# cambridge-mlg/RECOMBINER

Measured on AMD Instinct MI355X. Metric: INRs trained/sec (whole node) + PSNR@bpp vs reference, CIFAR-10, higher is better.
Workload: dtype bf16

## Files before the change

include/rcb.h:

```cpp
#ifndef RCB_H_
#define RCB_H_

#include <stdint.h>

#ifdef __cplusplus
extern "C" {
#endif

#define RCB_VERSION 406
#define RCB_OK 0
#define RCB_ERR_ARG (-1)
#define RCB_ERR_SHAPE (-2)
#define RCB_ERR_UNSUPPORTED (-3)
#define RCB_KL_SLOTS 1024
#define RCB_KL_FX_SCALE 16777216.0

typedef void* rcb_stream_t;

int rcb_version(void);
const char* rcb_last_error_string(void);
#define RCB_STRUCT_SIREN_DESC 0
#define RCB_STRUCT_LEVEL 1
#define RCB_STRUCT_LEVEL_BWD 2
#define RCB_STRUCT_ADAM_CFG 3
#define RCB_STRUCT_ADAM_TENSOR 4
#define RCB_STRUCT_REC_DESC 5
int64_t rcb_struct_bytes(int32_t which);

typedef struct {
  int32_t n_rows;
  int32_t samples;
  int32_t n_pix;
  int32_t fourier_dim;
  int32_t pe_dim;
  int32_t n_hidden;
  int32_t hidden;
  int32_t out_dim;
  int64_t xf_inr_stride;
  int64_t w_row_stride;
  float   w0;
  int32_t precision;
  int32_t pe_bf16;
// ... 98 lines not shown
  void* next_out_bf16;
  int64_t next_ld_bf16;
  uint64_t rng_seed;
  const int64_t* rng_step_dev;
  int64_t rng_step_add;
  uint32_t rng_stream;
  uint32_t eps_from_rng;
  uint64_t rng_group_offset;
  void* next_out_lo;
  float* sample_sum_ws;
  const int32_t* col_map;
} rcb_level_bwd;

int rcb_posterior_bwd(const rcb_level_bwd* lv, const rcb_adam_cfg* adam, rcb_stream_t stream);

int rcb_adam_flat(float* p, const float* g, float* m, float* v, int64_t n, const rcb_adam_cfg* cfg,
                  rcb_stream_t stream);

#define RCB_ADAM_MAX_TENSORS 16
typedef struct {
  float* p;
  const float* g;
  float* m;
  float* v;
  int64_t n;
} rcb_adam_tensor;
int rcb_adam_multi(const rcb_adam_tensor* tensors, int32_t count, const rcb_adam_cfg* cfg, rcb_stream_t stream);

int rcb_debug_generic_kernels_only(int32_t on);

#define RCB_ATRANS_MAX_LAYERS 8
#define RCB_ATRANS_PLAN_HEAD 12
int64_t rcb_atrans_pack_elems(int32_t n_layers, const int32_t* sizes);
int rcb_atrans_pack(const float* const* A, int32_t n_layers, const int32_t* sizes, void* packed, int32_t want_lo,
                    rcb_stream_t stream);
int rcb_atrans_plan(int64_t rows, int32_t n_layers, const int32_t* sizes, int32_t n_cu, int32_t* plan, int32_t max_ints);
int rcb_atrans_apply(const float* x, int64_t ld_x, const void* x_hi, const void* x_lo, int64_t ld_x16, float* out,
                     int64_t ld_out, int64_t rows, int32_t n_layers, const int32_t* sizes, const void* packed, int32_t transpose,
                     int32_t terms, const int32_t* plan_dev, const int32_t* plan_head, float* workspace, rcb_stream_t stream);
int64_t rcb_atrans_workspace_floats(int64_t rows, int32_t n_layers, const int32_t* sizes, const int32_t* plan_head);
int64_t rcb_atrans_wgrad_narrow_workspace(int32_t L, int32_t n_slabs);
int rcb_atrans_wgrad_narrow(const float* h, const void* h_hi, const void* h_lo, int64_t ld_h, const float* d, const void* d_hi,
                            const void* d_lo, int64_t ld_d, int64_t rows, int32_t L, float* dA, float* workspace,
                            int32_t n_slabs, rcb_stream_t stream);

int rcb_step_begin(const float* adam_table, int64_t n_steps, const int64_t* step, float* dyn, int64_t* kl_slots,
                   rcb_stream_t stream);
int rcb_step_end(const float* sse, int32_t n_sse, double mse_scale, const int64_t* kl_slots, double* mse_log,
                 double* kl_log, int64_t n_log, int64_t* step, int64_t* aux_counter ,
                 rcb_stream_t stream);

#define RCB_MOM_FX_SCALE 1073741824.0
#define RCB_MOM_FX_LO_SCALE 4294967296.0
int rcb_col_moments(const float* loc, const float* log_scale, int32_t rows, int32_t cols, int64_t* out_fx,
                    rcb_stream_t stream);

#define RCB_REC_EXACT 0
#define RCB_REC_FAST 1

typedef struct rcb_rec_desc {
  const float* loc;
  const float* scale;
  const float* p_loc;
  const float* p_scale;
  int32_t rows, cols;
  const float* const* tables_t;
// ... 82 lines not shown
```

recombiner_amd/_lib.py:

```python
import ctypes as C
import os

import torch

_HERE = os.path.dirname(os.path.abspath(__file__))
LIB_PATH = os.environ.get("RCB_LIB") or os.path.join(_HERE, "lib", "librcb_hip.so")

EXPORTS = ["rcb_version", "rcb_last_error_string", "rcb_struct_bytes", "rcb_siren_fwd", "rcb_siren_bwd", "rcb_siren_loss_bwd",
           "rcb_reparam_fwd", "rcb_gauss_kl", "rcb_beta_update", "rcb_posterior_bwd", "rcb_adam_flat",
           "rcb_col_moments", "rcb_rec_score_argmax", "rcb_rec_commit", "rcb_rec_workspace_bytes", "rcb_softplus_scale", "rcb_gauss_kl_colsum", "rcb_upconv_fwd",
           "rcb_upconv_dgrad", "rcb_upconv_wgrad", "rcb_upconv_wgrad_workspace", "rcb_adam_multi", "rcb_step_begin",
           "rcb_step_end", "rcb_upconv_weff_build", "rcb_upconv_weff_grad",
           "rcb_upconv_dgrad_partial_rows", "rcb_debug_generic_kernels_only", "rcb_philox_normal",
           "rcb_reparam_rng_fwd", "rcb_upconv_bwd_fused", "rcb_tile_gather", "rcb_tile_crop", "rcb_tile_fold",
           "rcb_window_gather", "rcb_window_fold", "rcb_siren_reduce_chunks", "rcb_phaseconv_pack", "rcb_phaseconv_pack_uint4",
           "rcb_phaseconv_fwd", "rcb_phaseconv_dgrad", "rcb_phaseconv_wgrad", "rcb_phaseconv_wgrad_workspace",
           "rcb_phase_bigweight", "rcb_phase_bigweight_grad", "rcb_atrans_pack_elems", "rcb_atrans_pack", "rcb_atrans_plan",
           "rcb_atrans_apply", "rcb_atrans_workspace_floats", "rcb_atrans_wgrad_narrow_workspace", "rcb_atrans_wgrad_narrow",
           "rcb_stage1_1d_fwd", "rcb_stage1_1d_dgrad", "rcb_stage1_1d_wgrad", "rcb_stage1_1d_wgrad_workspace",
           "rcb_reparam_hier_rng_fwd", "rcb_debug_siren_wave_tiles"]


class RcbError(RuntimeError):
    pass


class SirenDesc(C.Structure):
    _fields_ = [("n_rows", C.c_int32), ("samples", C.c_int32), ("n_pix", C.c_int32), ("fourier_dim", C.c_int32),
                ("pe_dim", C.c_int32), ("n_hidden", C.c_int32), ("hidden", C.c_int32), ("out_dim", C.c_int32),
                ("xf_inr_stride", C.c_int64), ("w_row_stride", C.c_int64), ("w0", C.c_float),
                ("precision", C.c_int32), ("pe_bf16", C.c_int32), ("dw_bf16", C.c_void_p), ("pixel_chunks", C.c_int32),
                ("xf_bf16", C.c_void_p), ("pe_grid_dims", C.c_int32), ("pe_patch_nums", C.c_int32 * 3),
                ("pe_patch_size", C.c_int32 * 3), ("dw_bf16_stride", C.c_int64), ("hidden_dims", C.c_int32 * 4),
                ("dw_lo", C.c_void_p), ("clock_probe", C.c_void_p)]


class Level(C.Structure):
    _fields_ = [("loc", C.c_void_p), ("log_scale", C.c_void_p), ("enc_sample", C.c_void_p),
                ("enc_mask", C.c_void_p), ("row_map", C.c_void_p), ("row_perm", C.c_void_p),
                ("col_map", C.c_void_p), ("eps", C.c_void_p), ("rows", C.c_int32), ("cols", C.c_int32),
                ("cols_out", C.c_int32), ("scale_is_sigma", C.c_int32), ("mu_sigma_ws", C.c_void_p)]


class RecDesc(C.Structure):
    _fields_ = [("loc", C.c_void_p), ("scale", C.c_void_p), ("p_loc", C.c_void_p), ("p_scale", C.c_void_p),
                ("rows", C.c_int32), ("cols", C.c_int32), ("tables_t", C.c_void_p), ("table_absmax", C.c_void_p),
                ("max_glen", C.c_int32), ("gumbel", C.c_void_p), ("gumbel_absmax", C.c_double),
                ("n_candidates", C.c_int32), ("job_row", C.c_void_p), ("job_start", C.c_void_p),
                ("job_glen", C.c_void_p), ("n_jobs", C.c_int32)]


class AdamTensor(C.Structure):
    _fields_ = [("p", C.c_void_p), ("g", C.c_void_p), ("m", C.c_void_p), ("v", C.c_void_p), ("n", C.c_int64)]


class AdamCfg(C.Structure):
    _fields_ = [("lr", C.c_float), ("beta1", C.c_float), ("beta2", C.c_float), ("eps", C.c_float),
                ("step", C.c_int32), ("dyn_scalars", C.c_void_p)]


class LevelBwd(C.Structure):
    _fields_ = [("loc", C.c_void_p), ("log_scale", C.c_void_p), ("enc_mask", C.c_void_p), ("p_loc", C.c_void_p),
                ("p_scale", C.c_void_p), ("p_scale_is_log", C.c_int32), ("beta", C.c_void_p),
                ("group_idx", C.c_void_p), ("n_groups", C.c_int32), ("kl_scalar", C.c_float),
                ("d_out", C.c_void_p), ("eps", C.c_void_p), ("member_ptr", C.c_void_p),
                ("member_idx", C.c_void_p), ("row_perm_inv", C.c_void_p), ("col_inv", C.c_void_p),
                ("rows", C.c_int32), ("cols", C.c_int32), ("cols_out", C.c_int32), ("samples", C.c_int32),
                ("g_loc", C.c_void_p), ("g_log_scale", C.c_void_p), ("m_loc", C.c_void_p), ("v_loc", C.c_void_p),
                ("m_ls", C.c_void_p), ("v_ls", C.c_void_p), ("kl_accum", C.c_void_p), ("kl_scalar_dev", C.c_void_p),
                ("next_out", C.c_void_p), ("next_eps", C.c_void_p), ("next_out_bf16", C.c_void_p),
                ("next_ld_bf16", C.c_int64), ("rng_seed", C.c_uint64), ("rng_step_dev", C.c_void_p),
                ("rng_step_add", C.c_int64), ("rng_stream", C.c_uint32), ("eps_from_rng", C.c_uint32),
                ("rng_group_offset", C.c_uint64), ("next_out_lo", C.c_void_p), ("sample_sum_ws", C.c_void_p), ("col_map", C.c_void_p)]


_lib = None
ABI_VERSION = 406
_MIRRORS = {0: SirenDesc, 1: Level, 2: LevelBwd, 3: AdamCfg, 4: AdamTensor, 5: RecDesc}


def load():
    global _lib
    if _lib is None:
        if not os.path.exists(LIB_PATH):
            raise RcbError(f"{LIB_PATH} not found: run `python -m recombiner_amd.build` (no CPU fallback exists)")
        lib = C.CDLL(LIB_PATH)
        lib.rcb_last_error_string.restype = C.c_char_p
        lib.rcb_upconv_wgrad_workspace.restype = C.c_int64
        lib.rcb_rec_workspace_bytes.restype = C.c_int64
        lib.rcb_phaseconv_pack_uint4.restype = C.c_int64
        lib.rcb_phaseconv_wgrad_workspace.restype = C.c_int64
        lib.rcb_stage1_1d_wgrad_workspace.restype = C.c_int64
        lib.rcb_atrans_pack_elems.restype = C.c_int64
        lib.rcb_atrans_wgrad_narrow_workspace.restype = C.c_int64
        lib.rcb_atrans_workspace_floats.restype = C.c_int64
        for name in EXPORTS:
            if not hasattr(lib, name):
                raise RcbError(f"{LIB_PATH} does not export {name}")
        lib.rcb_struct_bytes.restype = C.c_int64
        if lib.rcb_version() != ABI_VERSION:
            raise RcbError(f"{LIB_PATH} is ABI version {lib.rcb_version()}, this binding was written against {ABI_VERSION}: "
                           "rebuild with `python -m recombiner_amd.build --force`")
        for which, cls in _MIRRORS.items():
            if lib.rcb_struct_bytes(which) != C.sizeof(cls):
                raise RcbError(f"{cls.__name__}: the library's structure has {lib.rcb_struct_bytes(which)} bytes, the ctypes "
                               f"mirror {C.sizeof(cls)} -- _lib.py has drifted from include/rcb.h")
        _lib = lib
    return _lib


# ... 29 lines not shown
```

recombiner_amd/csrc/atrans.hip:

```cpp
#include "rcb_common.h"

#include <algorithm>
#include <type_traits>
#include <vector>

using namespace rcb;

namespace {

typedef __bf16 bf16x8 __attribute__((ext_vector_type(8)));
typedef float f32x16 __attribute__((ext_vector_type(16)));
typedef float f32x4 __attribute__((ext_vector_type(4)));

#ifndef ATRANS_DIAG
#define ATRANS_DIAG 0
#endif
#ifndef ATRANS_STAMPS
#define ATRANS_STAMPS 0
#endif
#ifndef ATRANS_SPREAD_PIN
#define ATRANS_SPREAD_PIN 1
#endif
constexpr int BM = 256, BK = 32, NT = 512, MAXL = RCB_ATRANS_MAX_LAYERS, MAXSEG = 7;
constexpr int XT_BYTES = BM * BK * 4;

__device__ __forceinline__ constexpr int rho(int r, int h) { return (r & 3) + 8 * (r >> 2) + 4 * h; }
__device__ __forceinline__ int xswz(int row, int c) { return row * 128 + ((c ^ ((row >> 1) & 7)) << 4); }
__device__ __forceinline__ int bswz(int row, int c) { return row * 64 + ((c ^ ((row >> 2) & 3)) << 4); }

typedef __attribute__((address_space(3))) void* lds_ptr_t;
__device__ __forceinline__ void dma16(const void* g, char* l) {
  __builtin_amdgcn_global_load_lds(g, (lds_ptr_t)l, 16, 0, 0);
}
__device__ __forceinline__ f32x16 mma(bf16x8 a, bf16x8 b, f32x16 c) {
#if ATRANS_DIAG == 4
  asm volatile("" ::"v"(a), "v"(b));
  return c;
#else
  return __builtin_amdgcn_mfma_f32_32x32x16_bf16(a, b, c, 0, 0, 0);
#endif
}
template <int N>
__device__ __forceinline__ void wait_vm() { asm volatile("s_waitcnt vmcnt(%0)" ::"n"(N) : "memory"); }
#if ATRANS_STAMPS
__device__ unsigned long long g_stamps[8][40][6];
#define STAMP(it, pt)                                                                 \
  do {                                                                               \
    if (blockIdx.x == 0 && (it) < 40) {                                              \
      const unsigned long long t_ = __builtin_amdgcn_s_memtime();                    \
      if (lane == 0) g_stamps[wave][it][pt] = t_;                                    \
    }                                                                                \
  } while (0)
#else
#define STAMP(it, pt)
#endif

struct AtArgs {
  const float* x;
  const __bf16* xh;
  const __bf16* xl;
  long long ld_x16;
  float* out;
  long long ld_x, ld_out, rows;
  int n_layers;
  int L[MAXL], Lp[MAXL], off[MAXL];
  const __bf16* bh[MAXL];
  const __bf16* bl[MAXL];
  const int4* segs;
  const int* seg_begin;
  int n_wg;
  int nt_out;
  float* ws;
  long long ld_ws;
};

template <int NCB, int TERMS>
struct Geo {
  static constexpr int NBW = (2 * NCB + 7) / 8;
  static constexpr int NDMA = 4 + NBW * (TERMS == 3 ? 2 : 1);
  static constexpr int BH_OFF = XT_BYTES;
  static constexpr int BT_BYTES = NCB * 32 * BK * 2;
  static constexpr int BL_OFF = BH_OFF + BT_BYTES;
  static constexpr int STAGE = BH_OFF + (TERMS == 3 ? 2 : 1) * BT_BYTES;
  static constexpr int NSTAGE = TERMS == 3 ? 2 : 3;
};
constexpr int LDS_MAX_BYTES = 3 * (XT_BYTES + MAXSEG * 32 * BK * 2);

template <int NCB, int TERMS, bool RAGGED, bool PLANES>
__device__ __forceinline__ void run_segment(const AtArgs& a, const int4 sg, const int4 sk, char* __restrict__ lds) {
  typedef Geo<NCB, TERMS> G;
  const int t = threadIdx.x, lane = t & 63;
  const int wave = __builtin_amdgcn_readfirstlane(t >> 6);
  const int l = sg.x, row0 = sg.y, cb0 = sg.z, ncb = sg.w;
  const int K = a.L[l], Lp = a.Lp[l];
  const int kc0 = sk.x, nk = sk.y - sk.x;
  const __bf16* __restrict__ bh = a.bh[l];
  const __bf16* __restrict__ bl = a.bl[l];
  const float* __restrict__ xl0 = PLANES ? nullptr : a.x + a.off[l];

  f32x16 acc[NCB];
#pragma unroll
  for (int i = 0; i < NCB; ++i)
#pragma unroll
    for (int q = 0; q < 16; ++q) acc[i][q] = 0.f;

  const float* xsrc[4];
  const __bf16* psrc[4];
  int xk[4];
#pragma unroll
  for (int i = 0; i < 4; ++i) {
    if (PLANES) {
      const int row = 32 * wave + 16 * (i & 1) + (lane >> 2);
      const int c = (lane & 3) ^ ((row >> 2) & 3);
      const long long gr = min((long long)row0 + row, a.rows - 1);
      psrc[i] = ((i >> 1) ? a.xl : a.xh) + gr * a.ld_x16 + a.off[l];
      xk[i] = 8 * c;
      xsrc[i] = nullptr;
    } else {
      const int row = 32 * wave + 8 * i + (lane >> 3);
      const int c = (lane & 7) ^ ((row >> 1) & 7);
      const long long gr = min((long long)row0 + row, a.rows - 1);
      xsrc[i] = xl0 + gr * a.ld_x;
      xk[i] = 4 * c;
      psrc[i] = nullptr;
    }
  }
  const __bf16* bsrc[G::NBW];
  const __bf16* bsrc2[G::NBW];
  int bdst[G::NBW];
#pragma unroll
  for (int j = 0; j < G::NBW; ++j) {
    const int d = min(wave + 8 * j, 2 * NCB - 1);
    const int row = 16 * d + (lane >> 2);
    const int c = (lane & 3) ^ ((row >> 2) & 3);
    const int grow = min(cb0 * 32 + row, Lp - 1);
    bsrc[j] = bh + (long long)grow * Lp + 8 * c;
    bsrc2[j] = bl + (long long)grow * Lp + 8 * c;
    bdst[j] = __builtin_amdgcn_readfirstlane(d * 1024);
  }
  auto issue_one = [&](int kc_, int i) {
    char* __restrict__ st = lds + (kc_ % G::NSTAGE) * G::STAGE;
    const int kc = ATRANS_DIAG == 2 ? 0 : kc0 + kc_;
    if (i < 4) {
      if (PLANES) {
        const int k = RAGGED ? 0 : min(kc * BK + xk[i], K - 8);
        dma16(psrc[i] + k, st + (i >> 1) * (XT_BYTES / 2) + (32 * wave + 16 * (i & 1)) * 64);
      } else {
        const int k = RAGGED ? 0 : min(kc * BK + xk[i], K - 4);
        dma16(xsrc[i] + k, st + (32 * wave + 8 * i) * 128);
      }
    } else if (TERMS == 3) {
      const int j = (i - 4) >> 1;
      if ((i - 4) & 1) dma16(bsrc2[j] + kc * BK, st + G::BL_OFF + bdst[j]);
      else dma16(bsrc[j] + kc * BK, st + G::BH_OFF + bdst[j]);
    } else {
      dma16(bsrc[i - 4] + kc * BK, st + G::BH_OFF + bdst[i - 4]);
    }
  };
  auto issue = [&](int kc) {
#pragma unroll
    for (int i = 0; i < G::NDMA; ++i) issue_one(kc, i);
  };

  const int frow = lane & 31, fh = lane >> 5;
  const int xrow = 32 * wave + frow;
  bf16x8 xh[2], xlo[2];
  f32x4 raw[4];
  auto x_read = [&](const char* __restrict__ st) {
    if (PLANES) {
#pragma unroll
      for (int q = 0; q < 4; ++q)
        if (TERMS >= 2 || q < 2)
          raw[q] = *reinterpret_cast<const f32x4*>(st + (q >> 1) * (XT_BYTES / 2) + bswz(xrow, 2 * (q & 1) + fh));
    } else {
#pragma unroll
      for (int q = 0; q < 4; ++q) raw[q] = *reinterpret_cast<const f32x4*>(st + xswz(xrow, 4 * (q >> 1) + 2 * fh + (q & 1)));
    }
  };
  auto x_convert = [&](int q) {
    if (PLANES) {
      if (q < 2) xh[q] = __builtin_bit_cast(bf16x8, raw[q]);
      else if (TERMS >= 2) xlo[q - 2] = __builtin_bit_cast(bf16x8, raw[q]);
      return;
    }
#pragma unroll
    for (int i = 0; i < 4; ++i) {
      const float v = raw[q][i];
      const __bf16 hb = (__bf16)v;
      xh[q >> 1][4 * (q & 1) + i] = hb;
      if (TERMS >= 2) xlo[q >> 1][4 * (q & 1) + i] = (__bf16)(v - (float)hb);
    }
  };
  constexpr int NBT = G::NDMA - 4;
  constexpr int CBR = (NCB - 1) / 2;
  auto compute = [&](const char* __restrict__ cur, const char* __restrict__ nxt, int kn, auto issue_c, auto pref_c) {
    constexpr bool ISSUE = decltype(issue_c)::value, PREF = decltype(pref_c)::value;
    bf16x8 b0 = *reinterpret_cast<const bf16x8*>(cur + G::BH_OFF + bswz(frow, fh));
    bf16x8 b1 = *reinterpret_cast<const bf16x8*>(cur + G::BH_OFF + bswz(frow, 2 + fh));
#pragma unroll
    for (int cb = 0; cb < NCB; ++cb) {
      const bf16x8 c0 = b0, c1 = b1;
      if (cb + 1 < NCB) {
        b0 = *reinterpret_cast<const bf16x8*>(cur + G::BH_OFF + bswz((cb + 1) * 32 + frow, fh));
        b1 = *reinterpret_cast<const bf16x8*>(cur + G::BH_OFF + bswz((cb + 1) * 32 + frow, 2 + fh));
      }
      acc[cb] = mma(xh[0], c0, acc[cb]);
// ... 19 lines not shown
        }
      }
#if ATRANS_SPREAD_PIN
      __builtin_amdgcn_sched_barrier(0);
#endif
    }
    if (PREF) {
      STAMP(kn - 2, 4);
#pragma unroll
      for (int q = 0; q < 4; ++q) x_convert(q);
    }
  };
  auto yes = std::integral_constant<bool, true>{};
  auto no = std::integral_constant<bool, false>{};

  if (RAGGED) {
    for (int kr = 0; kr < nk; ++kr) {
      const int kc = kc0 + kr;
      __syncthreads();
#pragma unroll
      for (int j = 0; j < G::NBW; ++j) {
        dma16(bsrc[j] + kc * BK, lds + G::BH_OFF + bdst[j]);
        if (TERMS == 3) dma16(bsrc2[j] + kc * BK, lds + G::BL_OFF + bdst[j]);
      }
#pragma unroll
      for (int i = 0; i < 4; ++i) {
        const int k0 = kc * BK + xk[i];
        if (PLANES) {
          const int row = 32 * wave + 16 * (i & 1) + (lane >> 2), pc = lane & 3;
          const bool rok = (long long)row0 + row < a.rows;
          bf16x8 v;
#pragma unroll
          for (int e = 0; e < 8; ++e) v[e] = (rok && k0 + e < K) ? psrc[i][k0 + e] : (__bf16)0.f;
          *reinterpret_cast<bf16x8*>(lds + (i >> 1) * (XT_BYTES / 2) + row * 64 + pc * 16) = v;
        } else {
          const int row = 32 * wave + 8 * i + (lane >> 3), pc = lane & 7;
          const bool rok = (long long)row0 + row < a.rows;
          f32x4 v;
#pragma unroll
          for (int e = 0; e < 4; ++e) v[e] = (rok && k0 + e < K) ? xsrc[i][k0 + e] : 0.f;
          *reinterpret_cast<f32x4*>(lds + row * 128 + pc * 16) = v;
        }
      }
      wait_vm<0>();
      __syncthreads();
      x_read(lds);
#pragma unroll
      for (int q = 0; q < 4; ++q) x_convert(q);
      compute(lds, lds, -1, no, no);
    }
    __syncthreads();
  } else if (G::NSTAGE == 2) {
    issue(0);
    for (int kc = 0; kc < nk; ++kc) {
      wait_vm<0>();
      __builtin_amdgcn_s_barrier();
      __builtin_amdgcn_sched_barrier(0);
      const char* cur = lds + (kc & 1) * G::STAGE;
      x_read(cur);
#pragma unroll
      for (int q = 0; q < 4; ++q) x_convert(q);
      if (kc + 1 < nk) compute(cur, cur, kc + 1, yes, no);
      else compute(cur, cur, -1, no, no);
    }
    __builtin_amdgcn_s_barrier();
  } else {
    issue(0);
// ... 5 lines not shown
    }
    x_read(lds);
#pragma unroll
    for (int q = 0; q < 4; ++q) x_convert(q);
    int kc = 0;
    for (; kc + 2 < nk; ++kc) {
      STAMP(kc, 0);
      wait_vm<G::NDMA>();
      STAMP(kc, 1);
      __builtin_amdgcn_s_barrier();
      __builtin_amdgcn_sched_barrier(0);
      STAMP(kc, 2);
      if (ATRANS_DIAG != 3) compute(lds + (kc % 3) * G::STAGE, lds + ((kc + 1) % 3) * G::STAGE, kc + 2, yes, yes);
      else issue(kc + 2);
      STAMP(kc, 5);
    }
    if (kc + 1 < nk) {
      wait_vm<G::NDMA>();
      __builtin_amdgcn_s_barrier();
      __builtin_amdgcn_sched_barrier(0);
      if (ATRANS_DIAG != 3) compute(lds + (kc % 3) * G::STAGE, lds + ((kc + 1) % 3) * G::STAGE, -1, no, yes);
      ++kc;
    }
    wait_vm<0>();
    __builtin_amdgcn_s_barrier();
    __builtin_amdgcn_sched_barrier(0);
    if (ATRANS_DIAG != 3) compute(lds + (kc % 3) * G::STAGE, lds, -1, no, no);
    __builtin_amdgcn_s_barrier();
  }

  const bool direct = sk.z < 0;
  float* __restrict__ ob = (direct ? a.out : a.ws + (long long)sk.z * a.rows * a.ld_ws) + a.off[l];
  const long long ldo = direct ? a.ld_out : a.ld_ws;
#pragma unroll
  for (int cb = 0; cb < NCB; ++cb) {
    if (cb < ncb && (ATRANS_DIAG != 1 || a.rows < 0)) {
      const int col = (cb0 + cb) * 32 + frow;
      if (col < K) {
#pragma unroll
        for (int q = 0; q < 16; ++q) {
          const long long row = (long long)row0 + 32 * wave + rho(q, fh);
          if (row < a.rows) {
            if (a.nt_out) __builtin_nontemporal_store(acc[cb][q], ob + row * ldo + col);
            else ob[row * ldo + col] = acc[cb][q];
          }
        }
      }
    }
  }
}

template <int TERMS, bool RAGGED, bool PLANES>
__device__ __forceinline__ void dispatch_upto4(const AtArgs& a, const int4 sg, const int4 sk, char* lds) {
  switch (sg.w) {
    case 1: run_segment<1, TERMS, RAGGED, PLANES>(a, sg, sk, lds); break;
    case 2: run_segment<2, TERMS, RAGGED, PLANES>(a, sg, sk, lds); break;
    case 3: run_segment<3, TERMS, RAGGED, PLANES>(a, sg, sk, lds); break;
    default: run_segment<4, TERMS, RAGGED, PLANES>(a, sg, sk, lds); break;
  }
}

template <int TERMS, bool RAGGED, bool PLANES>
__device__ __forceinline__ void dispatch_segment(const AtArgs& a, const int4 sg, const int4 sk, char* lds) {
  if constexpr (TERMS == 3) {
    if (sg.w > 4) {
      const int n1 = (sg.w + 1) / 2;
      dispatch_upto4<TERMS, RAGGED, PLANES>(a, make_int4(sg.x, sg.y, sg.z, n1), sk, lds);
      dispatch_upto4<TERMS, RAGGED, PLANES>(a, make_int4(sg.x, sg.y, sg.z + n1, sg.w - n1), sk, lds);
    } else {
      dispatch_upto4<TERMS, RAGGED, PLANES>(a, sg, sk, lds);
    }
    return;
  }
  switch (sg.w) {
    case 1: run_segment<1, TERMS, RAGGED, PLANES>(a, sg, sk, lds); break;
    case 2: run_segment<2, TERMS, RAGGED, PLANES>(a, sg, sk, lds); break;
    case 3: run_segment<3, TERMS, RAGGED, PLANES>(a, sg, sk, lds); break;
    case 4: run_segment<4, TERMS, RAGGED, PLANES>(a, sg, sk, lds); break;
    case 5: run_segment<5, TERMS, RAGGED, PLANES>(a, sg, sk, lds); break;
    case 6: run_segment<6, TERMS, RAGGED, PLANES>(a, sg, sk, lds); break;
    default: run_segment<7, TERMS, RAGGED, PLANES>(a, sg, sk, lds); break;
  }
}

template <int TERMS, bool PLANES>
__global__ void __launch_bounds__(NT, 2) atrans_kernel(AtArgs a) {
  extern __shared__ __attribute__((aligned(16))) char lds[];
  int id = blockIdx.x;
  if ((a.n_wg & 7) == 0) id = (id & 7) * (a.n_wg >> 3) + (id >> 3);
  const int s0 = a.seg_begin[id], s1 = a.seg_begin[id + 1];
  for (int s = s0; s < s1; ++s) {
    const int4 sg = a.segs[2 * s], sk = a.segs[2 * s + 1];
    if (a.L[sg.x] & 7) {
      if (sg.w > 1) run_segment<2, TERMS, true, PLANES>(a, sg, sk, lds);
      else run_segment<1, TERMS, true, PLANES>(a, sg, sk, lds);
    } else {
      dispatch_segment<TERMS, false, PLANES>(a, sg, sk, lds);
    }
  }
}

struct SlabArgs {
  const float* ws;
  float* out;
  long long rows, ld_ws, ld_out;
  int n_layers;
  int off[MAXL + 1], slabs[MAXL];
};

__global__ void __launch_bounds__(256) atrans_slab_sum_kernel(SlabArgs a) {
  const long long total = a.rows * a.off[a.n_layers];
  for (long long e = (long long)blockIdx.x * 256 + threadIdx.x; e < total; e += (long long)gridDim.x * 256) {
    const long long r = e / a.off[a.n_layers];
    const int c = (int)(e - r * a.off[a.n_layers]);
    int l = 0;
    while (l + 1 < a.n_layers && c >= a.off[l + 1]) ++l;
    float v = 0.f;
    for (int k = 0; k < a.slabs[l]; ++k) v += a.ws[((long long)k * a.rows + r) * a.ld_ws + c];
    a.out[r * a.ld_out + c] = v;
  }
}

struct PackArgs {
  const float* A[MAXL];
  int L[MAXL], Lp[MAXL], tile0[MAXL + 1];
  long long poff[MAXL];
  long long plane;
  __bf16* out;
  int n_layers, want_lo;
};
// ... 42 lines not shown
  {
    float v[4];
#pragma unroll
    for (int i = 0; i < 4; ++i) v[i] = tile[c4 + i][r];
    split_store(v, fwd_hi, fwd_lo, (long long)(j0 + r) * Lp + k0 + c4);
  }
}

inline int pad32(int v) { return (v + 31) / 32 * 32; }


struct Blk {
  int layer, cb, w, maxseg;
};

long long run_cost(const std::vector<Blk>& blks, int b0, int b1, std::vector<int4>* segs, int row0) {
  long long cost = 0;
  int i = b0;
  while (i < b1) {
    int j = i;
    while (j < b1 && blks[j].layer == blks[i].layer) ++j;
    const int n = j - i, ms = blks[i].maxseg, parts = (n + ms - 1) / ms;
    int done = 0;
    for (int p = 0; p < parts; ++p) {
      const int m = (n - done + (parts - p) - 1) / (parts - p);
      cost += (long long)m * blks[i].w + 6;
      if (segs) segs->push_back(make_int4(blks[i].layer, row0, blks[i + done].cb, m));
      done += m;
    }
    i = j;
  }
  return cost;
}

}

extern "C" int64_t rcb_atrans_pack_elems(int32_t n_layers, const int32_t* sizes) {
  if (!sizes || n_layers < 1 || n_layers > MAXL) return -1;
  int64_t plane = 0;
  for (int l = 0; l < n_layers; ++l) plane += (int64_t)pad32(sizes[l]) * pad32(sizes[l]);
  return 4 * plane;
}

extern "C" int rcb_atrans_pack(const float* const* A, int32_t n_layers, const int32_t* sizes, void* packed, int32_t want_lo,
                               rcb_stream_t stream) {
  RCB_REQUIRE(A && sizes && packed && n_layers >= 1 && n_layers <= MAXL, RCB_ERR_ARG, "atrans_pack: bad arguments (%d layers)", n_layers);
  RCB_REQUIRE((reinterpret_cast<uintptr_t>(packed) & 15) == 0, RCB_ERR_ARG, "atrans_pack: packed buffer must be 16-byte aligned");
  PackArgs a;
  memset(&a, 0, sizeof(a));
  long long plane = 0;
  int tiles = 0;
  for (int l = 0; l < n_layers; ++l) {
    RCB_REQUIRE(A[l] && sizes[l] >= 1, RCB_ERR_ARG, "atrans_pack: layer %d null / empty", l);
    a.A[l] = A[l];
    a.L[l] = sizes[l];
    a.Lp[l] = pad32(sizes[l]);
    a.poff[l] = plane;
    a.tile0[l] = tiles;
    plane += (long long)a.Lp[l] * a.Lp[l];
    tiles += (a.Lp[l] / 32) * (a.Lp[l] / 32);
  }
  a.tile0[n_layers] = tiles;
  a.plane = plane;
  a.out = reinterpret_cast<__bf16*>(packed);
  a.n_layers = n_layers;
  a.want_lo = want_lo;
  atrans_pack_kernel<<<tiles, 256, 0, (hipStream_t)stream>>>(a);
  RCB_LAUNCH_CHECK();
  return RCB_OK;
}

extern "C" int rcb_atrans_plan(int64_t rows, int32_t n_layers, const int32_t* sizes, int32_t n_cu, int32_t* plan,
                               int32_t max_ints) {
  RCB_REQUIRE(sizes && (plan || max_ints == 0) && n_layers >= 1 && n_layers <= MAXL && rows >= 1 && n_cu >= 1 && max_ints >= 0,
              RCB_ERR_ARG, "atrans_plan: bad arguments");
  std::vector<Blk> blks;
  for (int l = 0; l < n_layers; ++l) {
    RCB_REQUIRE(sizes[l] >= 1, RCB_ERR_ARG, "atrans_plan: layer %d empty", l);
    const int lp = pad32(sizes[l]);
    for (int cb = 0; cb < lp / 32; ++cb) blks.push_back(Blk{l, cb, lp / BK, (sizes[l] & 7) ? 2 : MAXSEG});
  }
  const int nb = (int)blks.size();
  const long long m_tiles = (rows + BM - 1) / BM;
  int R = (int)std::max<long long>(1, n_cu / m_tiles);
  R = std::min(R, (nb + 1) / 2);
  const int runs_full = (nb + MAXSEG - 1) / MAXSEG;
  int S = 1;
  if (m_tiles * runs_full * 2 <= n_cu) {
    S = (int)std::min<long long>(8, n_cu / (m_tiles * runs_full));
    R = runs_full;
  }
  long long lo = 0, hi = run_cost(blks, 0, nb, nullptr, 0);
  auto fits = [&](long long bound, std::vector<int>* cuts) {
    int b = 0, runs = 0;
    while (b < nb) {
      int e = b + 1;
      if (run_cost(blks, b, e, nullptr, 0) > bound) return false;
      while (e < nb && run_cost(blks, b, e + 1, nullptr, 0) <= bound) ++e;
      if (cuts) cuts->push_back(e);
      b = e;
      if (++runs > R) return false;
    }
    return true;
  };
  while (lo < hi) {
    const long long mid = (lo + hi) / 2;
    if (fits(mid, nullptr)) hi = mid; else lo = mid + 1;
  }
  std::vector<int> cuts;
  fits(hi, &cuts);
  const int runs = (int)cuts.size();
  std::vector<int4> segs;
  std::vector<int> begin;
  int slabs[MAXL];
  for (int l = 0; l < n_layers; ++l) slabs[l] = std::min(S, pad32(sizes[l]) / BK);
  for (long long mt = 0; mt < m_tiles; ++mt) {
    int b = 0;
    for (int ri = 0; ri < runs; ++ri) {
      std::vector<int4> run;
      run_cost(blks, b, cuts[ri], &run, (int)(mt * BM));
      b = cuts[ri];
      if (S == 1) {
        begin.push_back((int)segs.size() / 2);
        for (const int4& sg : run) {
          segs.push_back(sg);
          segs.push_back(make_int4(0, pad32(sizes[sg.x]) / BK, -1, 0));
        }
      } else {
        for (const int4& sg : run) {
          const int nc = pad32(sizes[sg.x]) / BK, sl = slabs[sg.x];
          for (int k = 0; k < sl; ++k) {
            begin.push_back((int)segs.size() / 2);
            segs.push_back(sg);
            segs.push_back(make_int4((int)((long long)k * nc / sl), (int)((long long)(k + 1) * nc / sl), k, 0));
          }
        }
      }
    }
  }
  begin.push_back((int)segs.size() / 2);
  const long long n_wg = (long long)begin.size() - 1;
  RCB_REQUIRE(n_wg < (1 << 24), RCB_ERR_SHAPE, "atrans_plan: %lld workgroups", n_wg);
  const long long head = ((RCB_ATRANS_PLAN_HEAD + n_wg + 1) + 3) / 4 * 4;
  const long long need = head + 4 * (long long)segs.size();
  RCB_REQUIRE(need < (1ll << 31), RCB_ERR_SHAPE, "atrans_plan: plan of %lld ints", need);
  if (max_ints == 0) return (int)need;
  if (need > max_ints) return rcb::fail(RCB_ERR_SHAPE, "atrans_plan: %lld ints needed, %d given", need, max_ints);
  memset(plan, 0, sizeof(int32_t) * head);
  plan[0] = (int32_t)n_wg;
  plan[1] = (int32_t)(segs.size() / 2);
  plan[2] = S;
  for (int l = 0; l < n_layers; ++l) plan[4 + l] = S == 1 ? 0 : slabs[l];
  for (size_t i = 0; i < begin.size(); ++i) plan[RCB_ATRANS_PLAN_HEAD + i] = begin[i];
  memcpy(plan + head, segs.data(), sizeof(int4) * segs.size());
  return (int)need;
}

extern "C" int rcb_atrans_apply(const float* x, int64_t ld_x, const void* x_hi, const void* x_lo, int64_t ld_x16, float* out,
                                int64_t ld_out, int64_t rows, int32_t n_layers, const int32_t* sizes, const void* packed,
                                int32_t transpose, int32_t terms, const int32_t* plan_dev, const int32_t* plan_head,
                                float* workspace, rcb_stream_t stream) {
  RCB_REQUIRE((x || x_hi) && out && sizes && packed && plan_dev && plan_head && n_layers >= 1 && n_layers <= MAXL && rows >= 1,
              RCB_ERR_ARG, "atrans_apply: bad arguments");
  const bool planes = x_hi != nullptr;
  RCB_REQUIRE(!planes || (x == nullptr && (x_lo != nullptr || terms == 1) && (ld_x16 & 7) == 0 &&
                          ((reinterpret_cast<uintptr_t>(x_hi) | reinterpret_cast<uintptr_t>(x_lo)) & 15) == 0),
              RCB_ERR_ARG, "atrans_apply: operand planes: give x_hi and x_lo (terms >= 2) INSTEAD of x, 16-byte aligned, row stride a multiple of 8");
  const int n_wg = plan_head[0], ksplit = plan_head[2];
  RCB_REQUIRE(n_wg >= 1 && ksplit >= 1 && ksplit <= 8 && (ksplit == 1 || workspace), RCB_ERR_ARG,
              "atrans_apply: plan head (workgroups %d, slices %d) / workspace", n_wg, ksplit);
  RCB_REQUIRE(terms >= 1 && terms <= 3, RCB_ERR_ARG, "atrans_apply: terms = %d (1..3)", terms);
  RCB_REQUIRE((reinterpret_cast<uintptr_t>(packed) & 15) == 0 && (reinterpret_cast<uintptr_t>(plan_dev) & 15) == 0, RCB_ERR_ARG,
              "atrans_apply: packed images / plan must be 16-byte aligned");
  AtArgs a;
  memset(&a, 0, sizeof(a));
  long long plane = 0, off = 0;
  for (int l = 0; l < n_layers; ++l) plane += (long long)pad32(sizes[l]) * pad32(sizes[l]);
  const __bf16* pk = reinterpret_cast<const __bf16*>(packed);
  long long poff = 0;
  for (int l = 0; l < n_layers; ++l) {
    a.L[l] = sizes[l];
    a.Lp[l] = pad32(sizes[l]);
    a.off[l] = (int)off;
    a.bh[l] = pk + (transpose ? plane : 0) + poff;
    a.bl[l] = pk + (transpose ? 3 : 2) * plane + poff;
    off += sizes[l];
    poff += (long long)a.Lp[l] * a.Lp[l];
  }
  RCB_REQUIRE((planes ? ld_x16 : ld_x) >= off && ld_out >= off, RCB_ERR_SHAPE, "atrans_apply: row strides %lld / %lld below %lld columns",
              (long long)(planes ? ld_x16 : ld_x), (long long)ld_out, off);
  if (planes)
    for (int l = 0; l < n_layers; ++l)
      RCB_REQUIRE((sizes[l] & 7) != 0 || (a.off[l] & 7) == 0, RCB_ERR_SHAPE, "atrans_apply: operand planes: layer %d starts at column %d (not a multiple of 8)", l, a.off[l]);
  a.x = x; a.out = out; a.ld_x = ld_x; a.ld_out = ld_out; a.rows = rows; a.n_layers = n_layers;
  a.xh = reinterpret_cast<const __bf16*>(x_hi);
  a.xl = reinterpret_cast<const __bf16*>(x_lo ? x_lo : x_hi);
  a.ld_x16 = ld_x16;
  a.nt_out = transpose ? 1 : 0;
  const long long head = ((RCB_ATRANS_PLAN_HEAD + (long long)n_wg + 1) + 3) / 4 * 4;
  a.seg_begin = plan_dev + RCB_ATRANS_PLAN_HEAD;
  a.segs = reinterpret_cast<const int4*>(plan_dev + head);
  a.n_wg = n_wg;
  a.ws = workspace;
  a.ld_ws = (off + 3) / 4 * 4;
  const int lds = LDS_MAX_BYTES;
  hipError_t e;
  auto go = [&](auto kfn) {
    e = hipFuncSetAttribute(reinterpret_cast<const void*>(kfn), hipFuncAttributeMaxDynamicSharedMemorySize, lds);
    if (e == hipSuccess) kfn<<<n_wg, NT, lds, (hipStream_t)stream>>>(a);
  };
  if (terms == 1) {
    if (planes) go(atrans_kernel<1, true>); else go(atrans_kernel<1, false>);
  } else if (terms == 2) {
    if (planes) go(atrans_kernel<2, true>); else go(atrans_kernel<2, false>);
  } else {
    if (planes) go(atrans_kernel<3, true>); else go(atrans_kernel<3, false>);
  }
  RCB_REQUIRE(e == hipSuccess, (int)e, "atrans_apply: hipFuncSetAttribute: %s", hipGetErrorString(e));
  RCB_LAUNCH_CHECK();
  if (ksplit > 1) {
    SlabArgs r;
    memset(&r, 0, sizeof(r));
    r.ws = workspace; r.out = out; r.rows = rows; r.ld_ws = a.ld_ws; r.ld_out = ld_out; r.n_layers = n_layers;
    for (int l = 0; l < n_layers; ++l) {
      r.off[l] = a.off[l];
      r.slabs[l] = plan_head[4 + l];
      RCB_REQUIRE(r.slabs[l] >= 1 && r.slabs[l] <= ksplit, RCB_ERR_ARG, "atrans_apply: plan head: %d slices for layer %d", r.slabs[l], l);
    }
    r.off[n_layers] = (int)off;
    long long blocks = (rows * off + 255) / 256;
    if (blocks > 4096) blocks = 4096;
    atrans_slab_sum_kernel<<<(int)blocks, 256, 0, (hipStream_t)stream>>>(r);
    RCB_LAUNCH_CHECK();
  }
  return RCB_OK;
}

extern "C" int64_t rcb_atrans_workspace_floats(int64_t rows, int32_t n_layers, const int32_t* sizes, const int32_t* plan_head) {
  if (!sizes || !plan_head || n_layers < 1 || n_layers > MAXL || rows < 1) return -1;
  if (plan_head[2] <= 1) return 0;
  long long off = 0;
  for (int l = 0; l < n_layers; ++l) off += sizes[l];
  return (int64_t)plan_head[2] * rows * ((off + 3) / 4 * 4);
}

namespace {
struct NarrowOp {
  const float* f;
  const __bf16* hi;
  const __bf16* lo;
// ... 61 lines not shown
    for (int u = 0; u < 8; ++u) v[u] = p[(sl + u) * st];
#pragma unroll
    for (int u = 0; u < 8; ++u) s += v[u];
  }
  for (; sl < n_slabs; ++sl) s += p[sl * st];
  dA[i] = s;
}
}

extern "C" int64_t rcb_atrans_wgrad_narrow_workspace(int32_t L, int32_t n_slabs) {
  if (L < 1 || n_slabs < 1) return -1;
  const int64_t nt = (L + 31) / 32;
  return (int64_t)n_slabs * nt * nt * 1024;
}

extern "C" int rcb_atrans_wgrad_narrow(const float* h, const void* h_hi, const void* h_lo, int64_t ld_h, const float* d,
                                       const void* d_hi, const void* d_lo, int64_t ld_d, int64_t rows, int32_t L, float* dA,
                                       float* workspace, int32_t n_slabs, rcb_stream_t stream) {
  RCB_REQUIRE(dA && workspace && rows >= 1 && L >= 1 && L <= 1024 && n_slabs >= 1 && n_slabs <= 4096, RCB_ERR_ARG,
              "atrans_wgrad_narrow: bad arguments (L = %d, slabs = %d)", L, n_slabs);
  RCB_REQUIRE((h != nullptr) != (h_hi != nullptr && h_lo != nullptr) && (d != nullptr) != (d_hi != nullptr && d_lo != nullptr), RCB_ERR_ARG,
              "atrans_wgrad_narrow: each operand either as fp32 rows or as a (hi, lo) pair of bf16 planes");
  RCB_REQUIRE(ld_h >= L && ld_d >= L, RCB_ERR_SHAPE, "atrans_wgrad_narrow: row strides below the layer size");
  const int nt = (L + 31) / 32;
  const NarrowOp hop{h, reinterpret_cast<const __bf16*>(h_hi), reinterpret_cast<const __bf16*>(h_lo), ld_h};
  const NarrowOp dop{d, reinterpret_cast<const __bf16*>(d_hi), reinterpret_cast<const __bf16*>(d_lo), ld_d};
  wgrad_narrow_kernel<<<nt * nt * n_slabs, 256, 0, (hipStream_t)stream>>>(hop, dop, rows, L, n_slabs, workspace);
  RCB_LAUNCH_CHECK();
  wgrad_narrow_sum_kernel<<<(L * L + 255) / 256, 256, 0, (hipStream_t)stream>>>(workspace, L, n_slabs, dA);
  RCB_LAUNCH_CHECK();
  return RCB_OK;
}

#if ATRANS_STAMPS
extern "C" int rcb_debug_atrans_stamps(unsigned long long* host, int32_t n) {
  if (n > 8 * 40 * 6) n = 8 * 40 * 6;
  hipError_t e = hipMemcpyFromSymbol(host, HIP_SYMBOL(g_stamps), sizeof(unsigned long long) * n);
  return (int)e;
}
#endif
```

Baseline: 71.78.

## Add a 128-row, 4-wave atrans tile form with longer segments when no k-split

Templates the atrans kernel on wave count. A 4-wave, 128-row-tile variant can now carry up to 14 column blocks per segment, or 7 with three terms. The planner picks this narrower-tile form whenever no k-split is chosen, aiming for more workgroups and better CU coverage on small row counts, and stores the tile height in the plan header. It also hoists output address math in the store loop and adds a debug override for the tile height. The cost is more template instantiations and a different LDS footprint and occupancy for each form.

```diff
diff --git a/include/rcb.h b/include/rcb.h
--- a/include/rcb.h
+++ b/include/rcb.h
@@ -7,7 +7,7 @@
 extern "C" {
 #endif
 
-#define RCB_VERSION 406
+#define RCB_VERSION 407
 #define RCB_OK 0
 #define RCB_ERR_ARG (-1)
 #define RCB_ERR_SHAPE (-2)
@@ -172,6 +172,7 @@
 #define RCB_ATRANS_MAX_LAYERS 8
 #define RCB_ATRANS_PLAN_HEAD 12
 int64_t rcb_atrans_pack_elems(int32_t n_layers, const int32_t* sizes);
+int rcb_debug_atrans_tiles(int32_t rows_per_tile);
 int rcb_atrans_pack(const float* const* A, int32_t n_layers, const int32_t* sizes, void* packed, int32_t want_lo,
                     rcb_stream_t stream);
 int rcb_atrans_plan(int64_t rows, int32_t n_layers, const int32_t* sizes, int32_t n_cu, int32_t* plan, int32_t max_ints);
diff --git a/recombiner_amd/_lib.py b/recombiner_amd/_lib.py
--- a/recombiner_amd/_lib.py
+++ b/recombiner_amd/_lib.py
@@ -18,7 +18,7 @@
            "rcb_phase_bigweight", "rcb_phase_bigweight_grad", "rcb_atrans_pack_elems", "rcb_atrans_pack", "rcb_atrans_plan",
            "rcb_atrans_apply", "rcb_atrans_workspace_floats", "rcb_atrans_wgrad_narrow_workspace", "rcb_atrans_wgrad_narrow",
            "rcb_stage1_1d_fwd", "rcb_stage1_1d_dgrad", "rcb_stage1_1d_wgrad", "rcb_stage1_1d_wgrad_workspace",
-           "rcb_reparam_hier_rng_fwd", "rcb_debug_siren_wave_tiles"]
+           "rcb_reparam_hier_rng_fwd", "rcb_debug_siren_wave_tiles", "rcb_debug_atrans_tiles"]
 
 
 class RcbError(RuntimeError):
@@ -75,7 +75,7 @@
 
 
 _lib = None
-ABI_VERSION = 406
+ABI_VERSION = 407
 _MIRRORS = {0: SirenDesc, 1: Level, 2: LevelBwd, 3: AdamCfg, 4: AdamTensor, 5: RecDesc}
 
 
diff --git a/recombiner_amd/csrc/atrans.hip b/recombiner_amd/csrc/atrans.hip
--- a/recombiner_amd/csrc/atrans.hip
+++ b/recombiner_amd/csrc/atrans.hip
@@ -21,8 +21,16 @@
 #ifndef ATRANS_SPREAD_PIN
 #define ATRANS_SPREAD_PIN 1
 #endif
-constexpr int BM = 256, BK = 32, NT = 512, MAXL = RCB_ATRANS_MAX_LAYERS, MAXSEG = 7;
-constexpr int XT_BYTES = BM * BK * 4;
+constexpr int BK = 32, MAXL = RCB_ATRANS_MAX_LAYERS;
+
+template <int NW>
+struct Form {
+  static constexpr int BM = 32 * NW, NT = 64 * NW;
+  static constexpr int XT = BM * BK * 4;
+  static constexpr int MAXSEG = NW == 8 ? 7 : 14;
+  static constexpr int T3MAX = NW == 8 ? 4 : 7;
+  static constexpr int LDS = std::max(3 * (XT + MAXSEG * 32 * BK * 2), 2 * (XT + 2 * T3MAX * 32 * BK * 2));
+};
 
 __device__ __forceinline__ constexpr int rho(int r, int h) { return (r & 3) + 8 * (r >> 2) + 4 * h; }
 __device__ __forceinline__ int xswz(int row, int c) { return row * 128 + ((c ^ ((row >> 1) & 7)) << 4); }
@@ -74,22 +82,24 @@
   long long ld_ws;
 };
 
-template <int NCB, int TERMS>
+template <int NW, int NCB, int TERMS>
 struct Geo {
-  static constexpr int NBW = (2 * NCB + 7) / 8;
+  static constexpr int XT = Form<NW>::XT;
+  static constexpr int NBW = (2 * NCB + NW - 1) / NW;
   static constexpr int NDMA = 4 + NBW * (TERMS == 3 ? 2 : 1);
-  static constexpr int BH_OFF = XT_BYTES;
+  static constexpr int BH_OFF = XT;
   static constexpr int BT_BYTES = NCB * 32 * BK * 2;
   static constexpr int BL_OFF = BH_OFF + BT_BYTES;
   static constexpr int STAGE = BH_OFF + (TERMS == 3 ? 2 : 1) * BT_BYTES;
   static constexpr int NSTAGE = TERMS == 3 ? 2 : 3;
 };
-constexpr int LDS_MAX_BYTES = 3 * (XT_BYTES + MAXSEG * 32 * BK * 2);
-
-template <int NCB, int TERMS, bool RAGGED, bool PLANES>
+
+template <int NCB, int NW, int TERMS, bool RAGGED, bool PLANES>
 __device__ __forceinline__ void run_segment(const AtArgs& a, const int4 sg, const int4 sk, char* __restrict__ lds) {
-  typedef Geo<NCB, TERMS> G;
-  const int t = threadIdx.x, lane = t & 63;
+  typedef Geo<NW, NCB, TERMS> G;
+  int t = threadIdx.x;
+  asm volatile("" : "+v"(t));
+  const int lane = t & 63;
   const int wave = __builtin_amdgcn_readfirstlane(t >> 6);
   const int l = sg.x, row0 = sg.y, cb0 = sg.z, ncb = sg.w;
   const int K = a.L[l], Lp = a.Lp[l];
@@ -130,7 +140,7 @@
   int bdst[G::NBW];
 #pragma unroll
   for (int j = 0; j < G::NBW; ++j) {
-    const int d = min(wave + 8 * j, 2 * NCB - 1);
+    const int d = min(wave + NW * j, 2 * NCB - 1);
     const int row = 16 * d + (lane >> 2);
     const int c = (lane & 3) ^ ((row >> 2) & 3);
     const int grow = min(cb0 * 32 + row, Lp - 1);
@@ -144,7 +154,7 @@
     if (i < 4) {
       if (PLANES) {
         const int k = RAGGED ? 0 : min(kc * BK + xk[i], K - 8);
-        dma16(psrc[i] + k, st + (i >> 1) * (XT_BYTES / 2) + (32 * wave + 16 * (i & 1)) * 64);
+        dma16(psrc[i] + k, st + (i >> 1) * (G::XT / 2) + (32 * wave + 16 * (i & 1)) * 64);
       } else {
         const int k = RAGGED ? 0 : min(kc * BK + xk[i], K - 4);
         dma16(xsrc[i] + k, st + (32 * wave + 8 * i) * 128);
@@ -171,7 +181,7 @@
 #pragma unroll
       for (int q = 0; q < 4; ++q)
         if (TERMS >= 2 || q < 2)
-          raw[q] = *reinterpret_cast<const f32x4*>(st + (q >> 1) * (XT_BYTES / 2) + bswz(xrow, 2 * (q & 1) + fh));
+          raw[q] = *reinterpret_cast<const f32x4*>(st + (q >> 1) * (G::XT / 2) + bswz(xrow, 2 * (q & 1) + fh));
     } else {
 #pragma unroll
       for (int q = 0; q < 4; ++q) raw[q] = *reinterpret_cast<const f32x4*>(st + xswz(xrow, 4 * (q >> 1) + 2 * fh + (q & 1)));
@@ -257,7 +267,7 @@
           bf16x8 v;
 #pragma unroll
           for (int e = 0; e < 8; ++e) v[e] = (rok && k0 + e < K) ? psrc[i][k0 + e] : (__bf16)0.f;
-          *reinterpret_cast<bf16x8*>(lds + (i >> 1) * (XT_BYTES / 2) + row * 64 + pc * 16) = v;
+          *reinterpret_cast<bf16x8*>(lds + (i >> 1) * (G::XT / 2) + row * 64 + pc * 16) = v;
         } else {
           const int row = 32 * wave + 8 * i + (lane >> 3), pc = lane & 7;
           const bool rok = (long long)row0 + row < a.rows;
@@ -329,6 +339,9 @@
   const bool direct = sk.z < 0;
   float* __restrict__ ob = (direct ? a.out : a.ws + (long long)sk.z * a.rows * a.ld_ws) + a.off[l];
   const long long ldo = direct ? a.ld_out : a.ld_ws;
+  const long long rw = (long long)row0 + 32 * wave;
+  const int nrow = (int)min(a.rows - rw, 32ll);
+  float* __restrict__ ow = ob + (rw + 4 * fh) * ldo + cb0 * 32 + frow;
 #pragma unroll
   for (int cb = 0; cb < NCB; ++cb) {
     if (cb < ncb && (ATRANS_DIAG != 1 || a.rows < 0)) {
@@ -336,52 +349,48 @@
       if (col < K) {
 #pragma unroll
         for (int q = 0; q < 16; ++q) {
-          const long long row = (long long)row0 + 32 * wave + rho(q, fh);
-          if (row < a.rows) {
-            if (a.nt_out) __builtin_nontemporal_store(acc[cb][q], ob + row * ldo + col);
-            else ob[row * ldo + col] = acc[cb][q];
+          const int r = rho(q, 0);
+          if (r + 4 * fh < nrow) {
+            float* p = ow + r * ldo + cb * 32;
+            if (a.nt_out) __builtin_nontemporal_store(acc[cb][q], p);
+            else *p = acc[cb][q];
           }
         }
       }
     }
-  }
-}
-
-template <int TERMS, bool RAGGED, bool PLANES>
-__device__ __forceinline__ void dispatch_upto4(const AtArgs& a, const int4 sg, const int4 sk, char* lds) {
-  switch (sg.w) {
-    case 1: run_segment<1, TERMS, RAGGED, PLANES>(a, sg, sk, lds); break;
-    case 2: run_segment<2, TERMS, RAGGED, PLANES>(a, sg, sk, lds); break;
-    case 3: run_segment<3, TERMS, RAGGED, PLANES>(a, sg, sk, lds); break;
-    default: run_segment<4, TERMS, RAGGED, PLANES>(a, sg, sk, lds); break;
-  }
-}
-
-template <int TERMS, bool RAGGED, bool PLANES>
+    __builtin_amdgcn_sched_barrier(0);
+  }
+}
+
+template <int N, int NW, int TERMS, bool RAGGED, bool PLANES>
+__device__ __forceinline__ void run_upto(const AtArgs& a, const int4 sg, const int4 sk, char* lds) {
+  if constexpr (N > 1) {
+    if (sg.w < N) {
+      run_upto<N - 1, NW, TERMS, RAGGED, PLANES>(a, sg, sk, lds);
+      return;
+    }
+  }
+  run_segment<N, NW, TERMS, RAGGED, PLANES>(a, sg, sk, lds);
+}
+
+template <int NW, int TERMS, bool PLANES>
 __device__ __forceinline__ void dispatch_segment(const AtArgs& a, const int4 sg, const int4 sk, char* lds) {
+  typedef Form<NW> F;
   if constexpr (TERMS == 3) {
-    if (sg.w > 4) {
+    if (sg.w > F::T3MAX) {
       const int n1 = (sg.w + 1) / 2;
-      dispatch_upto4<TERMS, RAGGED, PLANES>(a, make_int4(sg.x, sg.y, sg.z, n1), sk, lds);
-      dispatch_upto4<TERMS, RAGGED, PLANES>(a, make_int4(sg.x, sg.y, sg.z + n1, sg.w - n1), sk, lds);
+      run_upto<F::T3MAX, NW, TERMS, false, PLANES>(a, make_int4(sg.x, sg.y, sg.z, n1), sk, lds);
+      run_upto<F::T3MAX, NW, TERMS, false, PLANES>(a, make_int4(sg.x, sg.y, sg.z + n1, sg.w - n1), sk, lds);
     } else {
-      dispatch_upto4<TERMS, RAGGED, PLANES>(a, sg, sk, lds);
+      run_upto<F::T3MAX, NW, TERMS, false, PLANES>(a, sg, sk, lds);
     }
     return;
   }
-  switch (sg.w) {
-    case 1: run_segment<1, TERMS, RAGGED, PLANES>(a, sg, sk, lds); break;
-    case 2: run_segment<2, TERMS, RAGGED, PLANES>(a, sg, sk, lds); break;
-    case 3: run_segment<3, TERMS, RAGGED, PLANES>(a, sg, sk, lds); break;
-    case 4: run_segment<4, TERMS, RAGGED, PLANES>(a, sg, sk, lds); break;
-    case 5: run_segment<5, TERMS, RAGGED, PLANES>(a, sg, sk, lds); break;
-    case 6: run_segment<6, TERMS, RAGGED, PLANES>(a, sg, sk, lds); break;
-    default: run_segment<7, TERMS, RAGGED, PLANES>(a, sg, sk, lds); break;
-  }
-}
-
-template <int TERMS, bool PLANES>
-__global__ void __launch_bounds__(NT, 2) atrans_kernel(AtArgs a) {
+  run_upto<F::MAXSEG, NW, TERMS, false, PLANES>(a, sg, sk, lds);
+}
+
+template <int NW, int TERMS, bool PLANES>
+__global__ void __launch_bounds__(64 * NW, NW / 4) atrans_kernel(AtArgs a) {
   extern __shared__ __attribute__((aligned(16))) char lds[];
   int id = blockIdx.x;
   if ((a.n_wg & 7) == 0) id = (id & 7) * (a.n_wg >> 3) + (id >> 3);
@@ -389,10 +398,10 @@
   for (int s = s0; s < s1; ++s) {
     const int4 sg = a.segs[2 * s], sk = a.segs[2 * s + 1];
     if (a.L[sg.x] & 7) {
-      if (sg.w > 1) run_segment<2, TERMS, true, PLANES>(a, sg, sk, lds);
-      else run_segment<1, TERMS, true, PLANES>(a, sg, sk, lds);
+      if (sg.w > 1) run_segment<2, NW, TERMS, true, PLANES>(a, sg, sk, lds);
+      else run_segment<1, NW, TERMS, true, PLANES>(a, sg, sk, lds);
     } else {
-      dispatch_segment<TERMS, false, PLANES>(a, sg, sk, lds);
+      dispatch_segment<NW, TERMS, PLANES>(a, sg, sk, lds);
     }
   }
 }
@@ -501,6 +510,8 @@
   }
   return cost;
 }
+
+int g_tile_rows = 0;
 
 }
 
@@ -543,22 +554,27 @@
                                int32_t max_ints) {
   RCB_REQUIRE(sizes && (plan || max_ints == 0) && n_layers >= 1 && n_layers <= MAXL && rows >= 1 && n_cu >= 1 && max_ints >= 0,
               RCB_ERR_ARG, "atrans_plan: bad arguments");
+  int nb = 0;
+  for (int l = 0; l < n_layers; ++l) {
+    RCB_REQUIRE(sizes[l] >= 1, RCB_ERR_ARG, "atrans_plan: layer %d empty", l);
+    nb += pad32(sizes[l]) / 32;
+  }
+  const int runs_full = (nb + Form<8>::MAXSEG - 1) / Form<8>::MAXSEG;
+  const long long m_tiles8 = (rows + Form<8>::BM - 1) / Form<8>::BM;
+  int S = 1;
+  if (m_tiles8 * runs_full * 2 <= n_cu) S = (int)std::min<long long>(8, n_cu / (m_tiles8 * runs_full));
+  if (g_tile_rows == Form<4>::BM) S = 1;
+  const bool wide = g_tile_rows ? g_tile_rows == Form<4>::BM : S == 1;
+  const int BM = wide ? Form<4>::BM : Form<8>::BM, maxseg = wide ? Form<4>::MAXSEG : Form<8>::MAXSEG;
   std::vector<Blk> blks;
   for (int l = 0; l < n_layers; ++l) {
-    RCB_REQUIRE(sizes[l] >= 1, RCB_ERR_ARG, "atrans_plan: layer %d empty", l);
     const int lp = pad32(sizes[l]);
-    for (int cb = 0; cb < lp / 32; ++cb) blks.push_back(Blk{l, cb, lp / BK, (sizes[l] & 7) ? 2 : MAXSEG});
-  }
-  const int nb = (int)blks.size();
+    for (int cb = 0; cb < lp / 32; ++cb) blks.push_back(Blk{l, cb, lp / BK, (sizes[l] & 7) ? 2 : maxseg});
+  }
   const long long m_tiles = (rows + BM - 1) / BM;
   int R = (int)std::max<long long>(1, n_cu / m_tiles);
   R = std::min(R, (nb + 1) / 2);
-  const int runs_full = (nb + MAXSEG - 1) / MAXSEG;
-  int S = 1;
-  if (m_tiles * runs_full * 2 <= n_cu) {
-    S = (int)std::min<long long>(8, n_cu / (m_tiles * runs_full));
-    R = runs_full;
-  }
+  if (S > 1) R = runs_full;
   long long lo = 0, hi = run_cost(blks, 0, nb, nullptr, 0);
   auto fits = [&](long long bound, std::vector<int>* cuts) {
     int b = 0, runs = 0;
@@ -619,6 +635,7 @@
   plan[0] = (int32_t)n_wg;
   plan[1] = (int32_t)(segs.size() / 2);
   plan[2] = S;
+  plan[3] = BM;
   for (int l = 0; l < n_layers; ++l) plan[4 + l] = S == 1 ? 0 : slabs[l];
   for (size_t i = 0; i < begin.size(); ++i) plan[RCB_ATRANS_PLAN_HEAD + i] = begin[i];
   memcpy(plan + head, segs.data(), sizeof(int4) * segs.size());
@@ -635,9 +652,9 @@
   RCB_REQUIRE(!planes || (x == nullptr && (x_lo != nullptr || terms == 1) && (ld_x16 & 7) == 0 &&
                           ((reinterpret_cast<uintptr_t>(x_hi) | reinterpret_cast<uintptr_t>(x_lo)) & 15) == 0),
               RCB_ERR_ARG, "atrans_apply: operand planes: give x_hi and x_lo (terms >= 2) INSTEAD of x, 16-byte aligned, row stride a multiple of 8");
-  const int n_wg = plan_head[0], ksplit = plan_head[2];
-  RCB_REQUIRE(n_wg >= 1 && ksplit >= 1 && ksplit <= 8 && (ksplit == 1 || workspace), RCB_ERR_ARG,
-              "atrans_apply: plan head (workgroups %d, slices %d) / workspace", n_wg, ksplit);
+  const int n_wg = plan_head[0], ksplit = plan_head[2], bm = plan_head[3];
+  RCB_REQUIRE(n_wg >= 1 && ksplit >= 1 && ksplit <= 8 && (ksplit == 1 || workspace) && (bm == Form<4>::BM || bm == Form<8>::BM),
+              RCB_ERR_ARG, "atrans_apply: plan head (workgroups %d, slices %d, tile rows %d) / workspace", n_wg, ksplit, bm);
   RCB_REQUIRE(terms >= 1 && terms <= 3, RCB_ERR_ARG, "atrans_apply: terms = %d (1..3)", terms);
   RCB_REQUIRE((reinterpret_cast<uintptr_t>(packed) & 15) == 0 && (reinterpret_cast<uintptr_t>(plan_dev) & 15) == 0, RCB_ERR_ARG,
               "atrans_apply: packed images / plan must be 16-byte aligned");
@@ -672,19 +689,23 @@
   a.n_wg = n_wg;
   a.ws = workspace;
   a.ld_ws = (off + 3) / 4 * 4;
-  const int lds = LDS_MAX_BYTES;
   hipError_t e;
-  auto go = [&](auto kfn) {
-    e = hipFuncSetAttribute(reinterpret_cast<const void*>(kfn), hipFuncAttributeMaxDynamicSharedMemorySize, lds);
-    if (e == hipSuccess) kfn<<<n_wg, NT, lds, (hipStream_t)stream>>>(a);
+  auto go = [&](auto form, auto kfn) {
+    typedef decltype(form) F;
+    e = hipFuncSetAttribute(reinterpret_cast<const void*>(kfn), hipFuncAttributeMaxDynamicSharedMemorySize, F::LDS);
+    if (e == hipSuccess) kfn<<<n_wg, F::NT, F::LDS, (hipStream_t)stream>>>(a);
   };
-  if (terms == 1) {
-    if (planes) go(atrans_kernel<1, true>); else go(atrans_kernel<1, false>);
-  } else if (terms == 2) {
-    if (planes) go(atrans_kernel<2, true>); else go(atrans_kernel<2, false>);
-  } else {
-    if (planes) go(atrans_kernel<3, true>); else go(atrans_kernel<3, false>);
-  }
+  auto pick = [&](auto form) {
+    constexpr int NW = decltype(form)::BM / 32;
+    if (terms == 1) {
+      if (planes) go(form, atrans_kernel<NW, 1, true>); else go(form, atrans_kernel<NW, 1, false>);
+    } else if (terms == 2) {
+      if (planes) go(form, atrans_kernel<NW, 2, true>); else go(form, atrans_kernel<NW, 2, false>);
+    } else {
+      if (planes) go(form, atrans_kernel<NW, 3, true>); else go(form, atrans_kernel<NW, 3, false>);
+    }
+  };
+  if (bm == Form<4>::BM) pick(Form<4>{}); else pick(Form<8>{});
   RCB_REQUIRE(e == hipSuccess, (int)e, "atrans_apply: hipFuncSetAttribute: %s", hipGetErrorString(e));
   RCB_LAUNCH_CHECK();
   if (ksplit > 1) {
@@ -812,6 +833,12 @@
   return RCB_OK;
 }
 
+extern "C" int rcb_debug_atrans_tiles(int32_t rows_per_tile) {
+  const int old = g_tile_rows;
+  if (rows_per_tile == 0 || rows_per_tile == Form<4>::BM || rows_per_tile == Form<8>::BM) g_tile_rows = rows_per_tile;
+  return old;
+}
+
 #if ATRANS_STAMPS
 extern "C" int rcb_debug_atrans_stamps(unsigned long long* host, int32_t n) {
   if (n > 8 * 40 * 6) n = 8 * 40 * 6;
```

After: 72.29, median of 6. Within noise of the previous version (+0.7%).
